# oramasearch/oramacore

Measured on NVIDIA H100. Metric: hybrid_search_qps_at_recall10_ge_0.99_1Mx768, higher is better.
Workload: dtype f32

## Files before the change

### include/oramacore_b200.h

```cpp
#ifndef ORAMACORE_B200_H
#define ORAMACORE_B200_H

#include <stddef.h>
#include <stdint.h>

#ifdef __cplusplus
extern "C" {
#endif

#define OC_OK 0
#define OC_ERR_INVALID (-1)
#define OC_ERR_CUDA (-2)
#define OC_ERR_OOM (-3)
#define OC_ERR_UNSUPPORTED (-4)
#define OC_ERR_COMM (-5)

#define OC_MAX_TOPK 1024u
#define OC_MAX_TOKENS 32u

#define OC_MODE_FULLTEXT 0
#define OC_MODE_VECTOR 1
#define OC_MODE_HYBRID 2

#define OC_DTYPE_F32 0
// ... 372 lines not shown
    float scan_ms;
    float bm25_ms;
    float fuse_ms;
    float comm_ms;
    uint32_t kernel_launches;
    uint32_t scan_launches;
    uint64_t scan_bytes;
    uint64_t bm25_postings;
    uint64_t h2d_bytes, d2h_bytes;
    uint32_t scan_tensor_core;
    uint32_t scan_unproven;
    uint32_t scan_variant;
    float scan_sweep_ms;
    float rerun_ms;
    uint32_t scan_rescored;
} oc_timing;
#define OC_SCAN_EXACT 0
#define OC_SCAN_TC_TF32 1
#define OC_SCAN_TC_BF16 4
#define OC_SCAN_TC_F16 5
int oc_last_timing(oc_ctx *ctx, oc_timing *out);
uint64_t oc_launch_count(oc_ctx *ctx);

#ifdef __cplusplus
}
#endif
#endif
```

### oramacore_b200/_lib.py

```python
from __future__ import annotations

import ctypes as C
import os
import subprocess

_HERE = os.path.dirname(os.path.abspath(__file__))
SO_PATH = os.environ.get("OC_SO_PATH") or os.path.join(_HERE, "liboramacore_b200.so")
CSRC = os.path.join(_HERE, "csrc")

OC_OK = 0
OC_MAX_TOPK = 1024
OC_COMM_ID_BYTES = 128
OC_GEO_EARTH_RADIUS_M = 6371000.0
OC_GEO_MAX_VERTICES = 2048
OC_RANGE_LO_OPEN = 1
OC_RANGE_HI_OPEN = 2
OC_FACET_UNIQUE = 1
OC_SCAN_EXACT = 0
OC_SCAN_TC_TF32 = 1
OC_SCAN_TC_BF16 = 4
OC_SCAN_TC_F16 = 5
OC_EMB_COMPACT_SHRINK = 1
OC_BATCHER_MIXED = 1
OC_WHERE_NONE, OC_WHERE_VARIANT, OC_WHERE_RANGE, OC_WHERE_GEO_RADIUS, OC_WHERE_GEO_POLYGON = 0, 1, 2, 3, 4
# ... 118 lines not shown

class ResolveQuery(C.Structure):
    _fields_ = [("exact", C.c_int), ("tolerance", C.c_int), ("field_boost", C.c_void_p), ("field_mask", C.c_void_p)]


STEM_FN = C.CFUNCTYPE(C.c_size_t, C.c_void_p, C.c_size_t, C.c_void_p, C.c_size_t, C.c_void_p)


class Timing(C.Structure):
    _fields_ = [("h2d_ms", C.c_float), ("device_ms", C.c_float), ("d2h_ms", C.c_float), ("scan_ms", C.c_float),
                ("bm25_ms", C.c_float), ("fuse_ms", C.c_float), ("comm_ms", C.c_float),
                ("kernel_launches", C.c_uint32), ("scan_launches", C.c_uint32), ("scan_bytes", C.c_uint64),
                ("bm25_postings", C.c_uint64), ("h2d_bytes", C.c_uint64), ("d2h_bytes", C.c_uint64),
                ("scan_tensor_core", C.c_uint32), ("scan_unproven", C.c_uint32),
                ("scan_variant", C.c_uint32), ("scan_sweep_ms", C.c_float), ("rerun_ms", C.c_float),
                ("scan_rescored", C.c_uint32)]

    def as_dict(self):
        return {n: getattr(self, n) for n, _ in self._fields_}


def build(force: bool = False) -> str:
    srcs = [os.path.join(CSRC, f) for f in os.listdir(CSRC) if f.endswith((".cu", ".cuh", ".h"))]
    srcs.append(os.path.join(_HERE, "..", "include", "oramacore_b200.h"))
    stale = (not os.path.exists(SO_PATH)) or any(os.path.getmtime(s) > os.path.getmtime(SO_PATH) for s in srcs)
    if force or stale:
        r = subprocess.run(["make", "-C", CSRC] + (["-B"] if force else []), capture_output=True, text=True)
        if r.returncode != 0:
            raise RuntimeError("nvcc build failed:\n" + r.stdout + r.stderr)
    return SO_PATH

# ... 160 lines not shown
```

### oramacore_b200/csrc/bm25.cuh

```cuda
#pragma once
#include "oc_common.cuh"

namespace oc {

#ifndef OC_BM25_TILE_ROWS
#define OC_BM25_TILE_ROWS 8192
#endif
constexpr uint32_t BM25_TILE = OC_BM25_TILE_ROWS;
#ifndef OC_BM25_THREADS
#define OC_BM25_THREADS 256
#endif
constexpr uint32_t BM25_THREADS = OC_BM25_THREADS;
constexpr uint32_t BM25_CHUNK = BM25_THREADS * 4;

struct PostingRaw {
    uint32_t row;
    uint16_t tf, len;
};
struct Posting {
    uint32_t row;
    float ntf;
};

struct TermDesc {
// ... 49 lines not shown
    Posting o;
    o.row = r.row;
    o.ntf = bm25_ntf(r.tf, r.len, avg, b, __fsub_rn(1.0f, b), 1.0f);
    out[i] = o;
}

__device__ __forceinline__ float bm25_sat(float S, float k, float kp1, float idf) {
    return __fdiv_rn(__fmul_rn(__fmul_rn(idf, kp1), S), __fadd_rn(k, S));
}
struct PreDesc {
    const Posting *src;
    Posting *dst;
    float *dense;
    uint32_t len;
    float weight, idf;
    uint32_t pad;
};
__device__ __forceinline__ bool f32_is_normal(float x) {
    const uint32_t e = (__float_as_uint(x) >> 23) & 0xffu;
    return e != 0u && e != 0xffu;
}

constexpr uint32_t BM25_CLASSES = 5;
struct Bm25Params {
    const TermDesc *terms;
    const TokenDesc *tokens;
    const QueryDesc *queries;
    const uint32_t *term_token;
    const uint32_t *seg;
    uint32_t n_queries, n_tiles;
    uint64_t n_rows;
// ... 12 lines not shown
    unsigned long long *tau;
    uint64_t *cand_key;
    float *cand_ft;
    uint32_t *cand_cnt;
    uint32_t *tile_count;
    float *tile_max, *tile_min;
    uint32_t tile_first;
    uint32_t *matched_bits;
    const uint32_t *perm;
    uint32_t cls_off[BM25_CLASSES];
    uint32_t cls_nq[BM25_CLASSES];
    uint32_t cls_q0[BM25_CLASSES];
    float *row_ft;
    const uint32_t *q_ok_slot;
    uint64_t ok_words;
};
__device__ __forceinline__ const uint32_t *row_ok_of(const uint32_t *bits, const uint32_t *slot, uint64_t words, uint32_t q) {
    return (bits && slot) ? bits + size_t(slot[q]) * words : bits;
}
__host__ __device__ __forceinline__ void bm25_item_decode(const Bm25Params &p, const uint32_t k, uint32_t &tile, uint32_t &q) {
    if (!p.perm) { tile = k / p.n_queries; q = k % p.n_queries; return; }
    uint32_t g = 0;
    while (g + 1 < BM25_CLASSES && k >= p.cls_off[g + 1]) g++;
    const uint32_t local = k - p.cls_off[g], nqg = p.cls_nq[g];
    tile = local / nqg;
    q = p.perm[p.cls_q0[g] + local % nqg];
}

__host__ __device__ inline size_t bm25_smem_bytes(bool multi, bool threshold, bool omc, uint32_t cap) {
    size_t b = size_t(BM25_TILE) * 4;
    if (multi || omc) b += size_t(BM25_TILE) * 4;
    if (threshold) b += size_t(BM25_TILE) * 4;
    b += size_t(BM25_TILE) / 8;
    b += size_t(cap) * 8;
    return b + 64;
}

constexpr uint32_t PRE_CHUNK = 4096;
__global__ void __launch_bounds__(256) bm25_precompute_kernel(const PreDesc *pre, const uint2 *items, float k,
                                                              const uint32_t *row_ok_bits) {
    const uint2 it = items[blockIdx.x];
    const PreDesc d = pre[it.x];
    const float kp1 = __fadd_rn(k, 1.0f);
    const uint32_t lo = it.y * PRE_CHUNK, hi = min(d.len, lo + PRE_CHUNK);
    const uint2 *src = reinterpret_cast<const uint2 *>(d.src);
    uint2 *dst = reinterpret_cast<uint2 *>(d.dst);
    for (uint32_t i = lo + threadIdx.x; i < hi; i += blockDim.x) {
        const uint2 r = __ldg(src + i);
        const float ntf = __fmul_rn(d.weight, __uint_as_float(r.y));
        float c = __int_as_float(0x7fc00000);
        if (f32_is_normal(ntf)) c = bm25_sat(ntf, k, kp1, d.idf);
        if (d.dense) {
            const bool ok = !row_ok_bits || ((row_ok_bits[r.x >> 5] >> (r.x & 31)) & 1u);
            if (ok && c == c) d.dense[r.x] = c;
        } else {
            dst[i] = make_uint2(r.x, __float_as_uint(c));
        }
    }
}

struct DfParams {
    const TermDesc *terms;
    const TokenDesc *tokens;
    uint32_t n_tokens, n_tiles;
    const uint32_t *seg;
    const uint32_t *row_ok_bits;
    unsigned int *df;
    const uint32_t *tok_ok_slot;
    uint64_t ok_words;
};
__global__ void __launch_bounds__(BM25_THREADS) bm25_df_kernel(const DfParams p) {
    __shared__ uint8_t flag[BM25_TILE];
// ... 350 lines not shown

__host__ __device__ inline size_t bm25_tile2_smem_bytes(bool threshold, bool omc, uint32_t cap) {
    size_t b = size_t(BM25_TILE) * 4;
    if (omc) b += size_t(BM25_TILE) * 4;
    if (threshold) b += size_t(BM25_TILE) * 4;
    b += size_t(BM25_TILE) / 8;
    b += size_t(cap) * 8;
    return b + 64;
}

struct ItemTok {
    const void *ptr;
    uint32_t n;
    uint32_t flags;
    float w, idf;
    uint32_t bit, pad;
};
constexpr uint32_t BM25_FLAT_TOK = 4;
__global__ void __launch_bounds__(256) bm25_flatten_kernel(const Bm25Params p, ItemTok *flat) {
    const TermDesc *terms = p.terms; const TokenDesc *tokens = p.tokens; const QueryDesc *queries = p.queries;
    const uint32_t *seg = p.seg;
    const uint32_t n_tiles = p.n_tiles, n_queries = p.n_queries;
    const uint64_t gid = uint64_t(blockIdx.x) * blockDim.x + threadIdx.x;
    const uint64_t total = uint64_t(n_tiles) * n_queries * BM25_FLAT_TOK;
    if (gid >= total) return;
    const uint32_t j = uint32_t(gid % BM25_FLAT_TOK);
    const uint64_t item = gid / BM25_FLAT_TOK;
    uint32_t tile, q;
    bm25_item_decode(p, uint32_t(item), tile, q);
    const QueryDesc qd = queries[q];
    ItemTok it{};
    if (j < qd.token_end - qd.token_begin) {
        const TokenDesc tk = tokens[qd.token_begin + j];
        it.idf = tk.idf; it.bit = tk.bit;
        if (tk.term_end > tk.term_begin) {
            const TermDesc td = terms[tk.term_begin];
            it.flags = td.flags; it.w = td.weight;
            if (td.flags & TD_DENSE) {
                it.ptr = reinterpret_cast<const float *>(td.ptr) + size_t(tile) * BM25_TILE;
                it.n = td.len ? BM25_TILE : 0;
            } else {
                const uint32_t *sg = seg + size_t(tk.term_begin) * (n_tiles + 1);
                const uint32_t lo = sg[tile], hi = sg[tile + 1];
                it.ptr = reinterpret_cast<const uint2 *>(td.ptr) + lo;
                it.n = hi - lo;
            }
        }
    }
    flat[gid] = it;
}

template <bool THRESH, bool OMC, bool ROWFT = false>
__global__ void __launch_bounds__(BM25_THREADS, 1024 / BM25_THREADS) bm25_tile2_kernel(const Bm25Params p, const ItemTok *flat, unsigned int *work_counter) {
    extern __shared__ __align__(16) uint8_t smem[];
    float *score = reinterpret_cast<float *>(smem);
// ... 331 lines not shown
    const unsigned long long key = make_key(s, row);
    if (key <= tau) return;
    const uint32_t slot = atomicAdd(s_cnt, 1u);
    if (slot < cap) tbuf[slot] = key;
}
__device__ __forceinline__ bool t3_find(const uint2 *pp, uint32_t n, uint32_t row, uint32_t *payload) {
    uint32_t lo = 0, hi = n;
    while (lo < hi) { const uint32_t m = (lo + hi) >> 1; if (__ldg(&pp[m].x) < row) lo = m + 1; else hi = m; }
    if (lo < n) { const uint2 r = __ldg(pp + lo); if (r.x == row) { *payload = r.y; return true; } }
    return false;
}
__device__ __noinline__ float t3_fold(const ItemTok *tab, const uint32_t *bm, const uint32_t j, const uint2 rec, const uint32_t l,
                                         const float k, const float kp1) {
    constexpr uint32_t W = BM25_TILE / 32;
    const uint32_t w = l >> 5, bit = 1u << (l & 31u);
    float s = 0.f;
#pragma unroll 1
    for (uint32_t i = 0; i < BM25_FLAT_TOK; i++) {
        const uint32_t ni = tab[i].n;
        if (ni == 0) continue;
        const uint32_t fi = tab[i].flags;
        float ci;
        if (fi & TD_DENSE) ci = __ldg(reinterpret_cast<const float *>(tab[i].ptr) + l);
        else {
            uint32_t pay = rec.y;
            if (i != j) {
                if (!(bm[i * W + w] & bit)) continue;
                if (!t3_find(reinterpret_cast<const uint2 *>(tab[i].ptr), ni, rec.x, &pay)) continue;
            }
            if (fi & TD_PRE) ci = __uint_as_float(pay);
            else {
                const float ntf = __fmul_rn(tab[i].w, __uint_as_float(pay));
                ci = f32_is_normal(ntf) ? bm25_sat(ntf, k, kp1, tab[i].idf) : __int_as_float(0x7fc00000);
            }
        }
        if (ci == ci) s = __fadd_rn(s, ci);
    }
    return s;
// ... 51 lines not shown
            lmax = fmaxf(lmax, m4);
            if (!pos) lmin = fminf(lmin, fminf(fminf(sv[0], sv[1]), fminf(sv[2], sv[3])));
            if (m4 >= tau_f) t3_consider4(sv[0], sv[1], sv[2], sv[3], row0 + i * 4u, tau, tau_f, s_cnt, tbuf, cap);
        }
    };
    load(ca, 0);
#pragma unroll 1
    for (uint32_t h = 0; h < NB; h += 2) {
        load(cb, h + 1);
        fold(ca, h);
        if (h + 2 < NB) load(ca, h + 2);
        fold(cb, h + 1);
    }
}

__global__ void __launch_bounds__(BM25_THREADS, 1024 / BM25_THREADS) bm25_tile3_kernel(const Bm25Params p, const ItemTok *flat, unsigned int *work_counter) {
    constexpr uint32_t W = BM25_TILE / 32;
    extern __shared__ __align__(16) uint8_t smem[];
    uint32_t *touched = reinterpret_cast<uint32_t *>(smem);
    uint32_t *bm = touched + W;
    uint64_t *tbuf = reinterpret_cast<uint64_t *>(bm + BM25_FLAT_TOK * W);
    __shared__ uint32_t s_cnt2[2], s_matched2[2];
    __shared__ unsigned int s_maxo2[2], s_mino2[2];
    __shared__ ItemTok s_tab[2][BM25_FLAT_TOK];
    __shared__ uint32_t s_item_cur, s_item_next;

    const uint32_t tid = threadIdx.x;
    const float kp1 = __fadd_rn(p.k, 1.0f);
    const uint32_t n_items = p.n_tiles * p.n_queries;
    const uint32_t *okbits = p.row_ok_bits;

    for (uint32_t i = tid; i < (BM25_FLAT_TOK + 1) * W; i += BM25_THREADS) touched[i] = 0u;
    if (tid == 0) { s_item_cur = atomicAdd(work_counter, 1u); s_item_next = atomicAdd(work_counter, 1u); }
    if (tid < 2) { s_cnt2[tid] = 0; s_matched2[tid] = 0; s_maxo2[tid] = f32_ordered(0.f); s_mino2[tid] = f32_ordered(0.f); }
    __syncthreads();
    if (s_item_cur < n_items && tid < BM25_FLAT_TOK) s_tab[0][tid] = flat[size_t(s_item_cur) * BM25_FLAT_TOK + tid];
    unsigned long long tau_next = 0ull;
    if (s_item_cur < n_items) { uint32_t t0, q0; bm25_item_decode(p, s_item_cur, t0, q0); tau_next = __ldcg(p.tau + q0); }

    for (uint32_t par = 0;; par ^= 1u) {
        __syncthreads();
        const uint32_t item = s_item_cur;
        if (item >= n_items) break;
        const uint32_t next = s_item_next;
        uint32_t next2 = 0;
        if (tid == 0) next2 = atomicAdd(work_counter, 1u);
        uint32_t tile, q;
        bm25_item_decode(p, item, tile, q);
        const uint32_t row0 = tile * BM25_TILE;
        uint32_t *s_cnt = &s_cnt2[par];
        if (tid == 0) { s_cnt2[par ^ 1u] = 0; s_matched2[par ^ 1u] = 0; s_maxo2[par ^ 1u] = f32_ordered(0.f); s_mino2[par ^ 1u] = f32_ordered(0.f); }
        ItemTok nx{};
        if (next < n_items && tid < BM25_FLAT_TOK) nx = flat[size_t(next) * BM25_FLAT_TOK + tid];
        unsigned long long tau = tau_next;
        if (next < n_items) { uint32_t tn, qn; bm25_item_decode(p, next, tn, qn); tau_next = __ldcg(p.tau + qn); }

        const ItemTok *tab = s_tab[par];
        const float4 *d0 = nullptr, *d1 = nullptr, *d2 = nullptr, *d3 = nullptr;
        uint32_t nd = 0, n_list = 0;
        bool pos = p.k >= 0.f;
#pragma unroll
        for (uint32_t j = 0; j < BM25_FLAT_TOK; j++) {
            const uint32_t n = tab[j].n;
            if (n == 0) continue;
            pos = pos && tab[j].w >= 0.f && tab[j].idf >= 0.f;
            if (tab[j].flags & TD_DENSE) {
                const float4 *dp = reinterpret_cast<const float4 *>(tab[j].ptr);
                if (nd == 0) d0 = dp; else if (nd == 1) d1 = dp; else if (nd == 2) d2 = dp; else d3 = dp;
                nd++;
            } else n_list++;
// ... 9 lines not shown
#pragma unroll 1
                for (uint32_t j = 0; j < BM25_FLAT_TOK; j++) {
                    const uint32_t n = tab[j].n;
                    if (n == 0 || (tab[j].flags & TD_DENSE)) continue;
                    const uint2 *pp = reinterpret_cast<const uint2 *>(tab[j].ptr);
                    for (uint32_t pi = tid; pi < n; pi += BM25_THREADS) {
                        const uint32_t row = __ldg(&pp[pi].x);
                        if (okbits && !((__ldg(okbits + (row >> 5)) >> (row & 31u)) & 1u)) continue;
                        const uint32_t l = row - row0, bit = 1u << (l & 31u);
                        if (nd) atomicOr(&touched[l >> 5], bit);
                        if (use_bm) atomicOr(&bm[j * W + (l >> 5)], bit);
                    }
                }
                __syncthreads();
            }
            switch (nd) {
                case 0: break;
                case 1: t3_scan<1, BM25_THREADS>(d0, d1, d2, d3, touched, any_list, pos, row0, tid, tau, tau_f, s_cnt, tbuf, p.cap, matched, lmax, lmin); break;
                case 2: t3_scan<2, BM25_THREADS>(d0, d1, d2, d3, touched, any_list, pos, row0, tid, tau, tau_f, s_cnt, tbuf, p.cap, matched, lmax, lmin); break;
                case 3: t3_scan<3, BM25_THREADS>(d0, d1, d2, d3, touched, any_list, pos, row0, tid, tau, tau_f, s_cnt, tbuf, p.cap, matched, lmax, lmin); break;
                default: t3_scan<4, BM25_THREADS>(d0, d1, d2, d3, touched, any_list, pos, row0, tid, tau, tau_f, s_cnt, tbuf, p.cap, matched, lmax, lmin); break;
            }
            if (any_list) {
#pragma unroll 1
                for (uint32_t j = 0; j < BM25_FLAT_TOK; j++) {
                    const uint32_t n = tab[j].n;
                    if (n == 0 || (tab[j].flags & TD_DENSE)) continue;
                    const uint2 *pp = reinterpret_cast<const uint2 *>(tab[j].ptr);
                    for (uint32_t pi = tid; pi < n; pi += BM25_THREADS) {
                        const uint2 rec = __ldg(pp + pi);
                        const uint32_t l = rec.x - row0, w = l >> 5, bit = 1u << (l & 31u);
// ... 45 lines not shown
            c = p.n_keep;
            if (tid == 0) atomicMax(p.tau + q, (unsigned long long)tbuf[p.n_keep - 1]);
        }
        for (uint32_t i = tid; i < c; i += BM25_THREADS) {
            const uint64_t key = tbuf[i];
            p.cand_key[slot_base * p.n_keep + i] = key;
            p.cand_ft[slot_base * p.n_keep + i] = key_score(key);
        }
        if (tid == 0) {
            p.cand_cnt[slot_base] = c;
            p.tile_count[slot_base] = s_matched2[par];
            p.tile_max[slot_base] = f32_unordered(s_maxo2[par]);
            p.tile_min[slot_base] = f32_unordered(s_mino2[par]);
        }
        if (tid < BM25_FLAT_TOK) s_tab[par ^ 1u][tid] = nx;
        if (tid == 0) { s_item_cur = next; s_item_next = next2; }
    }
}

constexpr uint32_t BW_WARPS = 6, BW_CAP = 256;
struct __align__(16) WarpScratch {
    uint32_t touched[BM25_TILE / 32];
    uint32_t bm[BM25_FLAT_TOK * (BM25_TILE / 32)];
    uint64_t tbuf[BW_CAP];
    ItemTok tab[BM25_FLAT_TOK];
    uint32_t cnt, pad[3];
};
__device__ __noinline__ unsigned long long warp_keep_top(uint64_t *buf, const uint32_t count, const uint32_t n, const uint32_t lane) {
    constexpr uint32_t PER = BW_CAP / 32;
    unsigned long long k[PER];
#pragma unroll
    for (uint32_t u = 0; u < PER; u++) k[u] = lane + 32u * u < count ? buf[lane + 32u * u] : 0ull;
    __syncwarp();
    unsigned long long mine = 0ull, last = 0ull;
    for (uint32_t r = 0; r < n; r++) {
        unsigned long long m = k[0];
#pragma unroll
        for (uint32_t u = 1; u < PER; u++) m = k[u] > m ? k[u] : m;
        for (int o = 16; o > 0; o >>= 1) {
            const unsigned long long om = __shfl_xor_sync(0xffffffffu, m, o);
            m = om > m ? om : m;
// ... 9 lines not shown
    return last;
}
__global__ void __launch_bounds__(BW_WARPS * 32, 5) bm25_warp_kernel(const Bm25Params p, const ItemTok *flat, unsigned int *work_counter) {
    constexpr uint32_t W = BM25_TILE / 32;
    extern __shared__ __align__(16) uint8_t smem[];
    const uint32_t lane = threadIdx.x & 31u;
    WarpScratch &ws = reinterpret_cast<WarpScratch *>(smem)[threadIdx.x >> 5];
    uint32_t *touched = ws.touched, *bm = ws.bm;
    const ItemTok *tab = ws.tab;
    const float kp1 = __fadd_rn(p.k, 1.0f);
    const uint32_t n_items = p.n_tiles * p.n_queries;
    const uint32_t *okbits = p.row_ok_bits;

    for (uint32_t i = lane; i < W; i += 32) touched[i] = 0u;
    for (uint32_t i = lane; i < BM25_FLAT_TOK * W; i += 32) bm[i] = 0u;
    if (lane == 0) ws.cnt = 0u;
    uint32_t item = 0, next = 0;
    if (lane == 0) { item = atomicAdd(work_counter, 1u); next = atomicAdd(work_counter, 1u); }
    item = __shfl_sync(0xffffffffu, item, 0); next = __shfl_sync(0xffffffffu, next, 0);
    ItemTok cur{};
    if (item < n_items && lane < BM25_FLAT_TOK) cur = flat[size_t(item) * BM25_FLAT_TOK + lane];
    unsigned long long tau_next = 0ull;
    if (item < n_items) { uint32_t t0, q0; bm25_item_decode(p, item, t0, q0); tau_next = __ldcg(p.tau + q0); }

    while (item < n_items) {
        uint32_t next2 = 0;
        if (lane == 0) next2 = atomicAdd(work_counter, 1u);
        uint32_t tile, q;
        bm25_item_decode(p, item, tile, q);
        const uint32_t row0 = tile * BM25_TILE;
        if (lane < BM25_FLAT_TOK) ws.tab[lane] = cur;
        ItemTok nx{};
        if (next < n_items && lane < BM25_FLAT_TOK) nx = flat[size_t(next) * BM25_FLAT_TOK + lane];
        unsigned long long tau = tau_next;
        if (next < n_items) { uint32_t tn, qn; bm25_item_decode(p, next, tn, qn); tau_next = __ldcg(p.tau + qn); }
        __syncwarp();

        const float4 *d0 = nullptr, *d1 = nullptr, *d2 = nullptr, *d3 = nullptr;
        uint32_t nd = 0, n_list = 0;
        bool pos = p.k >= 0.f;
#pragma unroll
        for (uint32_t j = 0; j < BM25_FLAT_TOK; j++) {
            const uint32_t n = tab[j].n;
            if (n == 0) continue;
            pos = pos && tab[j].w >= 0.f && tab[j].idf >= 0.f;
            if (tab[j].flags & TD_DENSE) {
                const float4 *dp = reinterpret_cast<const float4 *>(tab[j].ptr);
                if (nd == 0) d0 = dp; else if (nd == 1) d1 = dp; else if (nd == 2) d2 = dp; else d3 = dp;
                nd++;
// ... 10 lines not shown
#pragma unroll 1
                for (uint32_t j = 0; j < BM25_FLAT_TOK; j++) {
                    const uint32_t n = tab[j].n;
                    if (n == 0 || (tab[j].flags & TD_DENSE)) continue;
                    const uint2 *pp = reinterpret_cast<const uint2 *>(tab[j].ptr);
                    for (uint32_t pi = lane; pi < n; pi += 32) {
                        const uint32_t row = __ldg(&pp[pi].x);
                        if (okbits && !((__ldg(okbits + (row >> 5)) >> (row & 31u)) & 1u)) continue;
                        const uint32_t l = row - row0, bit = 1u << (l & 31u);
                        if (nd) atomicOr(&touched[l >> 5], bit);
                        if (use_bm) atomicOr(&bm[j * W + (l >> 5)], bit);
                    }
                }
                __syncwarp();
            }
            switch (nd) {
                case 0: break;
                case 1: t3_scan<1, 32>(d0, d1, d2, d3, touched, any_list, pos, row0, lane, tau, tau_f, &ws.cnt, ws.tbuf, BW_CAP, matched, lmax, lmin); break;
                case 2: t3_scan<2, 32>(d0, d1, d2, d3, touched, any_list, pos, row0, lane, tau, tau_f, &ws.cnt, ws.tbuf, BW_CAP, matched, lmax, lmin); break;
                case 3: t3_scan<3, 32>(d0, d1, d2, d3, touched, any_list, pos, row0, lane, tau, tau_f, &ws.cnt, ws.tbuf, BW_CAP, matched, lmax, lmin); break;
                default: t3_scan<4, 32>(d0, d1, d2, d3, touched, any_list, pos, row0, lane, tau, tau_f, &ws.cnt, ws.tbuf, BW_CAP, matched, lmax, lmin); break;
            }
            if (any_list) {
#pragma unroll 1
                for (uint32_t j = 0; j < BM25_FLAT_TOK; j++) {
                    const uint32_t n = tab[j].n;
                    if (n == 0 || (tab[j].flags & TD_DENSE)) continue;
                    const uint2 *pp = reinterpret_cast<const uint2 *>(tab[j].ptr);
                    for (uint32_t pi = lane; pi < n; pi += 32) {
                        const uint2 rec = __ldg(pp + pi);
                        const uint32_t l = rec.x - row0, w = l >> 5, bit = 1u << (l & 31u);
// ... 47 lines not shown
            p.tile_count[slot_base] = matched;
            p.tile_max[slot_base] = lmax;
            p.tile_min[slot_base] = lmin;
            ws.cnt = 0u;
        }
        if (lane < BM25_FLAT_TOK && nx.n) {
            const char *pf = reinterpret_cast<const char *>(nx.ptr);
            const uint32_t bytes = (nx.flags & TD_DENSE) ? 1024u : min(nx.n * 8u, 1024u);
            for (uint32_t o = 0; o < bytes; o += 128u) asm volatile("prefetch.global.L1 [%0];" ::"l"(pf + o));
        }
        cur = nx;
        item = next;
        next = __shfl_sync(0xffffffffu, next2, 0);
        __syncwarp();
    }
}

struct PointParams {
    const TermDesc *terms; const TokenDesc *tokens; const QueryDesc *queries;
    uint32_t n_queries, v_stride;
    const uint32_t *v_row;
    const uint32_t *row_ok_bits;
    float k;
    int threshold;
    float *v_ft; uint8_t *v_present;
    const uint32_t *q_ok_slot;
    uint64_t ok_words;
};
__device__ __forceinline__ bool posting_find(const TermDesc &td, uint32_t row, uint32_t *payload) {
    const uint2 *pp = reinterpret_cast<const uint2 *>(td.ptr);
// ... 134 lines not shown
```

### oramacore_b200/csrc/capi.cu

```cuda
#include <cuda_runtime.h>

#include <cub/device/device_radix_sort.cuh>
#include <cub/device/device_scan.cuh>

#include <algorithm>
#include <atomic>
#include <chrono>
#include <cmath>
#include <cstdarg>
#include <cstdio>
#include <cstring>
#include <limits>
#include <map>
#include <memory>
#include <mutex>
#include <utility>
#include <string>
#include <unordered_map>
#include <unordered_set>
#include <vector>

#include "bm25.cuh"
#include "comm.h"
#include "dense_cache.h"
// ... 2494 lines not shown
    Slot<FacetSliceDev> s_fslices;
    Slot<TermDesc> s_terms;
    Slot<TokenDesc> s_tokens;
    Slot<QueryDesc> s_queries;
    Slot<PreDesc> s_pre;
    Slot<SortEntry> s_sent;
    Slot<SortQuery> s_sq;
    Slot<uint8_t> s_salt;
    Bm25Params bp{};
    FuseParams fp{};
    size_t fuse_smem = 0;
    const uint32_t *row_ok = nullptr;
    float *min_hint_dev = nullptr;
    unsigned int *tile_counter = nullptr;
    bool did_comm = false;
    size_t o_sc = 0, o_n = 0, o_cnt = 0, o_min = 0, o_gflag = 0, out_bytes = 0, o_resc = 0;
    uint8_t *dout = nullptr;
    uint64_t *d_doc = nullptr;
    float *d_score = nullptr;
    uint32_t *d_n = nullptr;
};

static int upload(const Packer &pk, HostBuf &hb, DevBuf &db, cudaStream_t st) {
    OCTRY(hb.ensure(pk.total + 256));
    OCTRY(db.ensure(pk.total + 256));
    pk.fill(hb.p);
    size_t run0 = 0;
    for (size_t i = 0; i <= pk.segs.size(); i++) {
        const bool brk = i == pk.segs.size() || pk.segs[i].direct;
        if (brk) {
            const size_t end = i == pk.segs.size() ? pk.total : pk.segs[i].off;
// ... 324 lines not shown
        size_t slot = (h ^ (h >> 29)) & (cap_t - 1);
        while (tab_v[slot] != 0xffffffffu && !(tab_k[slot].a == key.a && tab_k[slot].b == key.b)) slot = (slot + 1) & (cap_t - 1);
        if (tab_v[slot] == 0xffffffffu) {
            tab_k[slot] = key; tab_v[slot] = (uint32_t)uniq.size();
            uniq.push_back({e, 0, key}); distinct += terms[e].len;
        }
        uniq[tab_v[slot]].uses++;
        e_to_u[e] = tab_v[slot];
        walked += terms[e].len;
    }
    const char *share_env = getenv("OC_BM25_SHARE");
    const bool share_off = share_env && !strcmp(share_env, "off"), share_force = share_env && !strcmp(share_env, "force");
    const char *dense_env = getenv("OC_BM25_DENSE");
    const char *t2_env = getenv("OC_BM25_TILE2");
    const bool dense_on = !k.any_multi && !(dense_env && dense_env[0] == '0') && !share_off && !(t2_env && t2_env[0] == '0');
    const uint64_t rows_pad = uint64_t(k.n_tiles) * BM25_TILE;
    const uint64_t dense_min = std::max<uint64_t>(512, k.S->n_rows / 16);
    std::vector<uint8_t> u_dense(uniq.size(), 0);
    uint64_t n_dense = 0;
    if (dense_on)
        for (size_t u = 0; u < uniq.size(); u++)
            if (terms[uniq[u].first_e].len >= dense_min && (n_dense + 1) * rows_pad * 4 <= (size_t(8) << 30)) { u_dense[u] = 1; n_dense++; }
    uint64_t walked_l = 0, distinct_l = 0;
    for (size_t e = 0; e < terms.size(); e++)
        if (e_to_u[e] != 0xffffffffu && !u_dense[e_to_u[e]]) walked_l += terms[e].len;
    for (size_t u = 0; u < uniq.size(); u++) if (!u_dense[u]) distinct_l += terms[uniq[u].first_e].len;
    const bool lists = distinct_l && !share_off && (share_force || (walked_l >= 2 * distinct_l && walked_l >= (64u << 20))) &&
                       distinct_l * 8 <= (size_t(6) << 30);
    if (!lists && !n_dense) return OC_OK;
    std::vector<float *> u_arr(uniq.size(), nullptr);
    std::vector<uint8_t> u_kept(uniq.size(), 0);
    if (n_dense) {
        std::vector<DenseKey> keys;
        std::vector<uint32_t> key_u;
        uint32_t kb, bb;
        memcpy(&kb, &k.p->bm25_k, 4); memcpy(&bb, &k.p->bm25_b, 4);
        for (size_t u = 0; u < uniq.size(); u++)
            if (u_dense[u]) {
                keys.push_back(DenseKey{k.S->ident, uniq[u].key.a, uint32_t(uniq[u].key.b >> 32), uint32_t(uniq[u].key.b), kb, bb});
                key_u.push_back((uint32_t)u);
            }
        std::vector<float *> arr;
        std::vector<uint8_t> build;
        dense_cache_bind(k, keys, rows_pad * 4, arr, build);
        for (size_t i = 0; i < keys.size(); i++) { u_arr[key_u[i]] = arr[i]; u_kept[key_u[i]] = arr[i] && !build[i]; }
    }
    uint64_t n_buf = 0;
    for (size_t u = 0; u < uniq.size(); u++) n_buf += u_dense[u] && !u_arr[u];
    if (lists) OCTRY(c->pre_post.ensure(distinct_l * 8 + 64));
    if (n_buf) OCTRY(c->dense_buf.ensure(n_buf * rows_pad * 4));
    k.dense_bytes = n_buf * rows_pad * 4;
    uint64_t off = 0, doff = 0;
    std::vector<uint64_t> u_off(uniq.size());
    std::vector<uint8_t> u_used(uniq.size(), 0);
    for (size_t u = 0; u < uniq.size(); u++) {
        if (!u_dense[u] && !lists) continue;
        u_used[u] = 1;
        if (u_dense[u] && !u_arr[u]) { u_arr[u] = c->dense_buf.as<float>() + doff; doff += rows_pad; }
        if (u_kept[u]) continue;
        const TermDesc &td = terms[uniq[u].first_e];
        PreDesc pd{};
        pd.src = td.ptr; pd.len = td.len; pd.weight = td.weight;
        pd.idf = tokens[k.term_token[uniq[u].first_e]].idf;
        if (u_dense[u]) pd.dense = u_arr[u];
        else { u_off[u] = off; pd.dst = c->pre_post.as<Posting>() + off; off += td.len; }
        const uint32_t pi = (uint32_t)k.pre_descs.size();
        k.pre_descs.push_back(pd);
        for (uint32_t ch = 0; ch * PRE_CHUNK < td.len; ch++) k.pre_items.push_back(make_uint2(pi, ch));
    }
    for (size_t e = 0; e < terms.size(); e++) {
        const uint32_t u = e_to_u[e];
        if (u == 0xffffffffu || !u_used[u]) continue;
        if (u_dense[u]) { terms[e].ptr = reinterpret_cast<const Posting *>(u_arr[u]); terms[e].flags |= TD_DENSE; }
        else { terms[e].ptr = c->pre_post.as<Posting>() + u_off[u]; terms[e].flags |= TD_PRE; }
    }
    return OC_OK;
}

static void bm25_item_order(SearchCall &k) {
// ... 245 lines not shown
    if (k.pin_items) {
        pj->d_doc = s_pdoc.at(din);
        pj->d_pos = s_ppos.at(din);
        pj->d_cnt = s_pcnt.at(din);
    }
    const uint32_t n_keep = k.n_keep;
    k.cap = n_keep <= 32 ? std::max<uint32_t>(n_keep + BM25_CHUNK, BM25_SPARSE_MAX)
                         : next_pow2(std::max<uint32_t>(n_keep + BM25_CHUNK, BM25_SPARSE_MAX));
    k.o_sc = size_t(B) * k.limit * 8;
    k.o_n = k.o_sc + size_t(B) * k.limit * 4;
    k.o_cnt = (k.o_n + size_t(B) * 4 + 7) & ~size_t(7);
    k.o_min = k.o_cnt + size_t(B) * 8;
    k.o_gflag = k.o_min + size_t(B) * 4;
    k.out_bytes = k.o_gflag + ((size_t(B) + 3) & ~size_t(3));
    k.o_resc = k.out_bytes + ((size_t(B) + 3) & ~size_t(3));
    OCTRY(c->out_blob.ensure(k.out_bytes));
    OCTRY(c->h_out.ensure(k.o_resc + size_t(B) * 4));
    k.dout = c->out_blob.as<uint8_t>();
    k.d_doc = c->out_blob.as<uint64_t>();
    k.d_score = reinterpret_cast<float *>(k.dout + k.o_sc);
    k.d_n = reinterpret_cast<uint32_t *>(k.dout + k.o_n);
    return OC_OK;
}

static int bm25_stage(SearchCall &k) {
    oc_ctx *c = k.c; const oc_search_params *p = k.p;
    const uint32_t B = k.B, n_tiles = k.n_tiles, n_keep = k.n_keep; const StrSnap *S = k.S;
    const DevBuf &din = c->in_blob; cudaStream_t ps = k.side ? c->side : c->stream;
    CU(cudaEventRecord(c->ev[EV_BM0], ps));
    const uint64_t ok_words = uint64_t(n_tiles) * (BM25_TILE / 32);
    if (k.per_q) {
        OCTRY(c->row_ok.ensure(std::max<uint64_t>(ok_words, 1) * k.qfj.slots.size() * 4));
// ... 77 lines not shown
    bp.row_ok_bits = k.row_ok;
    if (k.per_q) { bp.q_ok_slot = k.qfj.d_q_slot_ft; bp.ok_words = ok_words; }
    bp.omc_row = p->omc ? k.omc_row_dev : k.s_omcr.at(din);
    bp.omc_mult = p->omc ? k.omc_row_mult_dev : k.s_omcrm.at(din);
    bp.n_omc = k.n_omc_rows;
    bp.v_row = nullptr;
    bp.v_stride = k.vlimit;
    bp.v_ft = nullptr; bp.v_present = nullptr;
    bp.min_hint = k.min_hint_dev;
    bp.n_keep = n_keep; bp.cap = k.cap;
    bp.tau = c->tau.as<unsigned long long>();
    bp.cand_key = c->cand_key.as<uint64_t>(); bp.cand_ft = c->cand_ft.as<float>();
    bp.cand_cnt = c->cand_cnt.as<uint32_t>(); bp.tile_count = c->tile_cnt.as<uint32_t>();
    bp.tile_max = c->tile_max.as<float>(); bp.tile_min = c->tile_min.as<float>();
    bp.tile_first = 0;
    if (!k.q_perm.empty()) {
        bp.perm = k.s_perm.at(din);
        uint32_t off = 0, q0 = 0;
        for (uint32_t g = 0; g < BM25_CLASSES; g++) {
            bp.cls_off[g] = off; bp.cls_nq[g] = k.cls_nq[g]; bp.cls_q0[g] = q0;
            off += k.cls_nq[g] * n_tiles; q0 += k.cls_nq[g];
        }
    }
    const SearchReq &r = k.r;
    if (r.fj || r.gj || r.sj) {
        OCTRY(c->mbits.ensure(size_t(B) * std::max<uint32_t>(n_tiles, 1) * (BM25_TILE / 32) * 4));
        bp.matched_bits = c->mbits.as<uint32_t>();
    }
    if (r.gj && n_tiles) {
        OCTRY(c->row_ft.ensure(size_t(B) * n_tiles * BM25_TILE * 4));
// ... 212 lines not shown
    CU(cudaEventRecord(c->ev[EV_FUSE0], c->stream));
    OCTRY(fuse_or_merge(k));
    CU(cudaEventRecord(c->ev[EV_FUSE1], c->stream));
    return OC_OK;
}

static int rerun_checks(SearchCall &k) {
    oc_ctx *c = k.c; const oc_search_params *p = k.p;
    const uint32_t B = k.B; uint8_t *h = c->h_out.as<uint8_t>();
    CU(cudaEventRecord(c->ev[EV_DEV], c->stream));
    CU(cudaMemcpyAsync(h, k.dout, k.out_bytes, cudaMemcpyDeviceToHost, c->stream));
    if (c->gemm_pending) {
        CU(cudaMemcpyAsync(h + k.out_bytes, c->g_flag.p, k.Bv, cudaMemcpyDeviceToHost, c->stream));
        CU(cudaMemcpyAsync(h + k.o_resc, c->g_resc.p, size_t(k.Bv) * 4, cudaMemcpyDeviceToHost, c->stream));
    }
    CU(cudaEventRecord(c->ev[EV_D2H], c->stream));
    CU(cudaStreamSynchronize(c->stream));
    {
        bool rerun = false;
        if (k.did_comm && k.has_v) for (uint32_t q = 0; q < B; q++) rerun = rerun || h[k.o_gflag + q] != 0;
        uint32_t redone = 0;
        if (c->gemm_pending || rerun) CU(cudaEventRecord(c->ev[EV_RR0], c->stream));
        if (c->gemm_pending) {
            const uint32_t Bv = k.Bv;
            uint64_t resc = 0;
            for (uint32_t q = 0; q < Bv; q++) resc += reinterpret_cast<const uint32_t *>(h + k.o_resc)[q];
            c->timing.scan_rescored = (uint32_t)(resc / Bv);
            OCTRY(fix_unproven(c, k.emb, h + k.out_bytes, Bv, k.vlimit, p->similarity, &redone));
        }
        if (redone || rerun) {
            c->gemm_pending = false;
            OCTRY(device_tail(k));
// ... 2172 lines not shown
```

Before: 159,500.

## Skip dense BM25 tile scans using per-tile score upper bounds and hit bitmaps

While building the dense BM25 term arrays, the precompute kernel now also records a nonzero bitmap and a per-tile maximum contribution. In the tile kernels, when the sum of dense bounds for a tile is below the query's current threshold tau, the full dense score scan is replaced by a popcount over the bitmaps to keep the match count. This avoids reading and scoring dense float arrays for tiles that cannot enter the top-k. The cost is extra atomics and memory during precompute, plus a stats readback. The tau handling also moves into shared memory.

```diff
diff --git a/include/oramacore_b200.h b/include/oramacore_b200.h
--- a/include/oramacore_b200.h
+++ b/include/oramacore_b200.h
@@ -410,6 +410,8 @@
     float scan_sweep_ms;
     float rerun_ms;
     uint32_t scan_rescored;
+    uint32_t bm25_dense_items;
+    uint32_t bm25_dense_skipped;
 } oc_timing;
 #define OC_SCAN_EXACT 0
 #define OC_SCAN_TC_TF32 1
diff --git a/oramacore_b200/_lib.py b/oramacore_b200/_lib.py
--- a/oramacore_b200/_lib.py
+++ b/oramacore_b200/_lib.py
@@ -156,7 +156,7 @@
                 ("bm25_postings", C.c_uint64), ("h2d_bytes", C.c_uint64), ("d2h_bytes", C.c_uint64),
                 ("scan_tensor_core", C.c_uint32), ("scan_unproven", C.c_uint32),
                 ("scan_variant", C.c_uint32), ("scan_sweep_ms", C.c_float), ("rerun_ms", C.c_float),
-                ("scan_rescored", C.c_uint32)]
+                ("scan_rescored", C.c_uint32), ("bm25_dense_items", C.c_uint32), ("bm25_dense_skipped", C.c_uint32)]
 
     def as_dict(self):
         return {n: getattr(self, n) for n, _ in self._fields_}
diff --git a/oramacore_b200/csrc/bm25.cuh b/oramacore_b200/csrc/bm25.cuh
--- a/oramacore_b200/csrc/bm25.cuh
+++ b/oramacore_b200/csrc/bm25.cuh
@@ -87,7 +87,7 @@
     float *dense;
     uint32_t len;
     float weight, idf;
-    uint32_t pad;
+    uint32_t n_tiles;
 };
 __device__ __forceinline__ bool f32_is_normal(float x) {
     const uint32_t e = (__float_as_uint(x) >> 23) & 0xffu;
@@ -130,6 +130,7 @@
     float *row_ft;
     const uint32_t *q_ok_slot;
     uint64_t ok_words;
+    uint32_t *dense_stat;
 };
 __device__ __forceinline__ const uint32_t *row_ok_of(const uint32_t *bits, const uint32_t *slot, uint64_t words, uint32_t q) {
     return (bits && slot) ? bits + size_t(slot[q]) * words : bits;
@@ -152,6 +153,16 @@
     return b + 64;
 }
 
+__host__ __device__ inline uint64_t bm25_dense_bytes(uint32_t n_tiles) {
+    const uint64_t rows_pad = uint64_t(n_tiles) * BM25_TILE;
+    return rows_pad * 4 + rows_pad / 8 + ((uint64_t(n_tiles) * 4 + 255) & ~uint64_t(255));
+}
+__host__ __device__ __forceinline__ const uint32_t *bm25_dense_bits(const float *arr, uint32_t n_tiles) {
+    return reinterpret_cast<const uint32_t *>(arr + size_t(n_tiles) * BM25_TILE);
+}
+__host__ __device__ __forceinline__ const float *bm25_dense_bound(const float *arr, uint32_t n_tiles) {
+    return reinterpret_cast<const float *>(bm25_dense_bits(arr, n_tiles) + size_t(n_tiles) * (BM25_TILE / 32));
+}
 constexpr uint32_t PRE_CHUNK = 4096;
 __global__ void __launch_bounds__(256) bm25_precompute_kernel(const PreDesc *pre, const uint2 *items, float k,
                                                               const uint32_t *row_ok_bits) {
@@ -160,18 +171,40 @@
     const float kp1 = __fadd_rn(k, 1.0f);
     const uint32_t lo = it.y * PRE_CHUNK, hi = min(d.len, lo + PRE_CHUNK);
     const uint2 *src = reinterpret_cast<const uint2 *>(d.src);
-    uint2 *dst = reinterpret_cast<uint2 *>(d.dst);
-    for (uint32_t i = lo + threadIdx.x; i < hi; i += blockDim.x) {
-        const uint2 r = __ldg(src + i);
-        const float ntf = __fmul_rn(d.weight, __uint_as_float(r.y));
-        float c = __int_as_float(0x7fc00000);
-        if (f32_is_normal(ntf)) c = bm25_sat(ntf, k, kp1, d.idf);
-        if (d.dense) {
+    if (!d.dense) {
+        uint2 *dst = reinterpret_cast<uint2 *>(d.dst);
+        for (uint32_t i = lo + threadIdx.x; i < hi; i += blockDim.x) {
+            const uint2 r = __ldg(src + i);
+            const float ntf = __fmul_rn(d.weight, __uint_as_float(r.y));
+            float c = __int_as_float(0x7fc00000);
+            if (f32_is_normal(ntf)) c = bm25_sat(ntf, k, kp1, d.idf);
+            dst[i] = make_uint2(r.x, __float_as_uint(c));
+        }
+        return;
+    }
+    uint32_t *bits = const_cast<uint32_t *>(bm25_dense_bits(d.dense, d.n_tiles));
+    unsigned int *bound = reinterpret_cast<unsigned int *>(const_cast<float *>(bm25_dense_bound(d.dense, d.n_tiles)));
+    const uint32_t lane = threadIdx.x & 31u;
+    for (uint32_t i0 = lo + (threadIdx.x - lane); i0 < hi; i0 += blockDim.x) {
+        const uint32_t i = i0 + lane;
+        uint32_t row = 0, v = 0;
+        if (i < hi) {
+            const uint2 r = __ldg(src + i);
+            const float ntf = __fmul_rn(d.weight, __uint_as_float(r.y));
+            float c = __int_as_float(0x7fc00000);
+            if (f32_is_normal(ntf)) c = bm25_sat(ntf, k, kp1, d.idf);
             const bool ok = !row_ok_bits || ((row_ok_bits[r.x >> 5] >> (r.x & 31)) & 1u);
-            if (ok && c == c) d.dense[r.x] = c;
-        } else {
-            dst[i] = make_uint2(r.x, __float_as_uint(c));
-        }
+            row = r.x;
+            if (ok && c == c) {
+                d.dense[row] = c;
+                if (c != 0.f) atomicOr(bits + (row >> 5), 1u << (row & 31u));
+                if (c > 0.f) v = __float_as_uint(c);
+            }
+        }
+        const uint32_t tile = row / BM25_TILE;
+        const uint32_t grp = __match_any_sync(0xffffffffu, tile);
+        const uint32_t m = __reduce_max_sync(grp, v);
+        if (m && lane == uint32_t(__ffs(grp) - 1)) atomicMax(bound + tile, m);
     }
 }
 
@@ -552,7 +585,8 @@
     uint32_t n;
     uint32_t flags;
     float w, idf;
-    uint32_t bit, pad;
+    uint32_t bit;
+    uint32_t bound;
 };
 constexpr uint32_t BM25_FLAT_TOK = 4;
 __global__ void __launch_bounds__(256) bm25_flatten_kernel(const Bm25Params p, ItemTok *flat) {
@@ -577,6 +611,7 @@
             if (td.flags & TD_DENSE) {
                 it.ptr = reinterpret_cast<const float *>(td.ptr) + size_t(tile) * BM25_TILE;
                 it.n = td.len ? BM25_TILE : 0;
+                if (td.len) it.bound = __float_as_uint(bm25_dense_bound(reinterpret_cast<const float *>(td.ptr), n_tiles)[tile]);
             } else {
                 const uint32_t *sg = seg + size_t(tk.term_begin) * (n_tiles + 1);
                 const uint32_t lo = sg[tile], hi = sg[tile + 1];
@@ -938,6 +973,11 @@
                                          const float k, const float kp1) {
     constexpr uint32_t W = BM25_TILE / 32;
     const uint32_t w = l >> 5, bit = 1u << (l & 31u);
+    static_assert(BM25_FLAT_TOK == 4, "t3_fold holds one dense contribution per flat token");
+    auto dense_at = [&](const uint32_t i) {
+        return (tab[i].n && (tab[i].flags & TD_DENSE)) ? __ldg(reinterpret_cast<const float *>(tab[i].ptr) + l) : 0.f;
+    };
+    const float cd0 = dense_at(0), cd1 = dense_at(1), cd2 = dense_at(2), cd3 = dense_at(3);
     float s = 0.f;
 #pragma unroll 1
     for (uint32_t i = 0; i < BM25_FLAT_TOK; i++) {
@@ -945,7 +985,7 @@
         if (ni == 0) continue;
         const uint32_t fi = tab[i].flags;
         float ci;
-        if (fi & TD_DENSE) ci = __ldg(reinterpret_cast<const float *>(tab[i].ptr) + l);
+        if (fi & TD_DENSE) ci = i == 0 ? cd0 : i == 1 ? cd1 : i == 2 ? cd2 : cd3;
         else {
             uint32_t pay = rec.y;
             if (i != j) {
@@ -1027,6 +1067,35 @@
     }
 }
 
+__device__ __forceinline__ float t3_dense_ub(const ItemTok *tab) {
+    float ub = 0.f;
+#pragma unroll
+    for (uint32_t j = 0; j < BM25_FLAT_TOK; j++)
+        if (tab[j].n && (tab[j].flags & TD_DENSE)) ub = __fadd_rn(ub, __uint_as_float(tab[j].bound));
+    return ub;
+}
+template <uint32_t STRIDE>
+__device__ __noinline__ uint32_t t3_count(const ItemTok *tab, const uint32_t *touched, const bool any_list, const uint32_t n_tiles,
+                                          const uint32_t tile, const uint32_t tid) {
+    constexpr uint32_t W = BM25_TILE / 32;
+    const uint32_t *bp[BM25_FLAT_TOK];
+#pragma unroll
+    for (uint32_t j = 0; j < BM25_FLAT_TOK; j++)
+        bp[j] = (tab[j].n && (tab[j].flags & TD_DENSE))
+                    ? bm25_dense_bits(reinterpret_cast<const float *>(tab[j].ptr) - size_t(tile) * BM25_TILE, n_tiles) + size_t(tile) * W
+                    : nullptr;
+    uint32_t m = 0;
+#pragma unroll 2
+    for (uint32_t w = tid; w < W; w += STRIDE) {
+        uint32_t u = 0;
+#pragma unroll
+        for (uint32_t j = 0; j < BM25_FLAT_TOK; j++) if (bp[j]) u |= __ldg(bp[j] + w);
+        if (any_list) u &= ~touched[w];
+        m += __popc(u);
+    }
+    return m;
+}
+
 __global__ void __launch_bounds__(BM25_THREADS, 1024 / BM25_THREADS) bm25_tile3_kernel(const Bm25Params p, const ItemTok *flat, unsigned int *work_counter) {
     constexpr uint32_t W = BM25_TILE / 32;
     extern __shared__ __align__(16) uint8_t smem[];
@@ -1037,6 +1106,8 @@
     __shared__ unsigned int s_maxo2[2], s_mino2[2];
     __shared__ ItemTok s_tab[2][BM25_FLAT_TOK];
     __shared__ uint32_t s_item_cur, s_item_next;
+    __shared__ uint32_t s_dense[2];
+    __shared__ unsigned long long s_tau2[2];
 
     const uint32_t tid = threadIdx.x;
     const float kp1 = __fadd_rn(p.k, 1.0f);
@@ -1044,12 +1115,15 @@
     const uint32_t *okbits = p.row_ok_bits;
 
     for (uint32_t i = tid; i < (BM25_FLAT_TOK + 1) * W; i += BM25_THREADS) touched[i] = 0u;
-    if (tid == 0) { s_item_cur = atomicAdd(work_counter, 1u); s_item_next = atomicAdd(work_counter, 1u); }
+    if (tid == 0) { s_item_cur = atomicAdd(work_counter, 1u); s_item_next = atomicAdd(work_counter, 1u); s_dense[0] = s_dense[1] = 0u; }
     if (tid < 2) { s_cnt2[tid] = 0; s_matched2[tid] = 0; s_maxo2[tid] = f32_ordered(0.f); s_mino2[tid] = f32_ordered(0.f); }
     __syncthreads();
     if (s_item_cur < n_items && tid < BM25_FLAT_TOK) s_tab[0][tid] = flat[size_t(s_item_cur) * BM25_FLAT_TOK + tid];
     unsigned long long tau_next = 0ull;
-    if (s_item_cur < n_items) { uint32_t t0, q0; bm25_item_decode(p, s_item_cur, t0, q0); tau_next = __ldcg(p.tau + q0); }
+    if (tid == 0) {
+        s_tau2[0] = 0ull;
+        if (s_item_cur < n_items) { uint32_t t0, q0; bm25_item_decode(p, s_item_cur, t0, q0); s_tau2[0] = __ldcg(p.tau + q0); }
+    }
 
     for (uint32_t par = 0;; par ^= 1u) {
         __syncthreads();
@@ -1065,8 +1139,8 @@
         if (tid == 0) { s_cnt2[par ^ 1u] = 0; s_matched2[par ^ 1u] = 0; s_maxo2[par ^ 1u] = f32_ordered(0.f); s_mino2[par ^ 1u] = f32_ordered(0.f); }
         ItemTok nx{};
         if (next < n_items && tid < BM25_FLAT_TOK) nx = flat[size_t(next) * BM25_FLAT_TOK + tid];
-        unsigned long long tau = tau_next;
-        if (next < n_items) { uint32_t tn, qn; bm25_item_decode(p, next, tn, qn); tau_next = __ldcg(p.tau + qn); }
+        unsigned long long tau = s_tau2[par];
+        if (tid == 0 && next < n_items) { uint32_t tn, qn; bm25_item_decode(p, next, tn, qn); tau_next = __ldcg(p.tau + qn); }
 
         const ItemTok *tab = s_tab[par];
         const float4 *d0 = nullptr, *d1 = nullptr, *d2 = nullptr, *d3 = nullptr;
@@ -1106,7 +1180,10 @@
                 }
                 __syncthreads();
             }
-            switch (nd) {
+            const bool skip = nd && pos && t3_dense_ub(tab) < tau_f;
+            if (nd && tid == 0) { s_dense[0]++; s_dense[1] += skip; }
+            if (skip) matched += t3_count<BM25_THREADS>(tab, touched, any_list, p.n_tiles, tile, tid);
+            else switch (nd) {
                 case 0: break;
                 case 1: t3_scan<1, BM25_THREADS>(d0, d1, d2, d3, touched, any_list, pos, row0, tid, tau, tau_f, s_cnt, tbuf, p.cap, matched, lmax, lmin); break;
                 case 2: t3_scan<2, BM25_THREADS>(d0, d1, d2, d3, touched, any_list, pos, row0, tid, tau, tau_f, s_cnt, tbuf, p.cap, matched, lmax, lmin); break;
@@ -1182,8 +1259,9 @@
             p.tile_min[slot_base] = f32_unordered(s_mino2[par]);
         }
         if (tid < BM25_FLAT_TOK) s_tab[par ^ 1u][tid] = nx;
-        if (tid == 0) { s_item_cur = next; s_item_next = next2; }
-    }
+        if (tid == 0) { s_item_cur = next; s_item_next = next2; s_tau2[par ^ 1u] = tau_next; }
+    }
+    if (tid == 0 && p.dense_stat && s_dense[0]) { atomicAdd(p.dense_stat, s_dense[0]); atomicAdd(p.dense_stat + 1, s_dense[1]); }
 }
 
 constexpr uint32_t BW_WARPS = 6, BW_CAP = 256;
@@ -1192,7 +1270,7 @@
     uint32_t bm[BM25_FLAT_TOK * (BM25_TILE / 32)];
     uint64_t tbuf[BW_CAP];
     ItemTok tab[BM25_FLAT_TOK];
-    uint32_t cnt, pad[3];
+    uint32_t cnt, dense_items, dense_skipped, pad;
 };
 __device__ __noinline__ unsigned long long warp_keep_top(uint64_t *buf, const uint32_t count, const uint32_t n, const uint32_t lane) {
     constexpr uint32_t PER = BW_CAP / 32;
@@ -1232,7 +1310,7 @@
 
     for (uint32_t i = lane; i < W; i += 32) touched[i] = 0u;
     for (uint32_t i = lane; i < BM25_FLAT_TOK * W; i += 32) bm[i] = 0u;
-    if (lane == 0) ws.cnt = 0u;
+    if (lane == 0) { ws.cnt = 0u; ws.dense_items = 0u; ws.dense_skipped = 0u; }
     uint32_t item = 0, next = 0;
     if (lane == 0) { item = atomicAdd(work_counter, 1u); next = atomicAdd(work_counter, 1u); }
     item = __shfl_sync(0xffffffffu, item, 0); next = __shfl_sync(0xffffffffu, next, 0);
@@ -1250,7 +1328,7 @@
         if (lane < BM25_FLAT_TOK) ws.tab[lane] = cur;
         ItemTok nx{};
         if (next < n_items && lane < BM25_FLAT_TOK) nx = flat[size_t(next) * BM25_FLAT_TOK + lane];
-        unsigned long long tau = tau_next;
+        unsigned long long tau = __shfl_sync(0xffffffffu, tau_next, 0);
         if (next < n_items) { uint32_t tn, qn; bm25_item_decode(p, next, tn, qn); tau_next = __ldcg(p.tau + qn); }
         __syncwarp();
 
@@ -1291,7 +1369,10 @@
                 }
                 __syncwarp();
             }
-            switch (nd) {
+            const bool skip = nd && pos && t3_dense_ub(tab) < tau_f;
+            if (nd && lane == 0) { ws.dense_items++; ws.dense_skipped += skip; }
+            if (skip) matched += t3_count<32>(tab, touched, any_list, p.n_tiles, tile, lane);
+            else switch (nd) {
                 case 0: break;
                 case 1: t3_scan<1, 32>(d0, d1, d2, d3, touched, any_list, pos, row0, lane, tau, tau_f, &ws.cnt, ws.tbuf, BW_CAP, matched, lmax, lmin); break;
                 case 2: t3_scan<2, 32>(d0, d1, d2, d3, touched, any_list, pos, row0, lane, tau, tau_f, &ws.cnt, ws.tbuf, BW_CAP, matched, lmax, lmin); break;
@@ -1369,6 +1450,7 @@
         next = __shfl_sync(0xffffffffu, next2, 0);
         __syncwarp();
     }
+    if (lane == 0 && p.dense_stat && ws.dense_items) { atomicAdd(p.dense_stat, ws.dense_items); atomicAdd(p.dense_stat + 1, ws.dense_skipped); }
 }
 
 struct PointParams {
diff --git a/oramacore_b200/csrc/capi.cu b/oramacore_b200/csrc/capi.cu
--- a/oramacore_b200/csrc/capi.cu
+++ b/oramacore_b200/csrc/capi.cu
@@ -2532,7 +2532,7 @@
     float *min_hint_dev = nullptr;
     unsigned int *tile_counter = nullptr;
     bool did_comm = false;
-    size_t o_sc = 0, o_n = 0, o_cnt = 0, o_min = 0, o_gflag = 0, out_bytes = 0, o_resc = 0;
+    size_t o_sc = 0, o_n = 0, o_cnt = 0, o_min = 0, o_gflag = 0, out_bytes = 0, o_resc = 0, o_dstat = 0;
     uint8_t *dout = nullptr;
     uint64_t *d_doc = nullptr;
     float *d_score = nullptr;
@@ -2887,13 +2887,13 @@
     const char *dense_env = getenv("OC_BM25_DENSE");
     const char *t2_env = getenv("OC_BM25_TILE2");
     const bool dense_on = !k.any_multi && !(dense_env && dense_env[0] == '0') && !share_off && !(t2_env && t2_env[0] == '0');
-    const uint64_t rows_pad = uint64_t(k.n_tiles) * BM25_TILE;
+    const uint64_t dbytes = bm25_dense_bytes(k.n_tiles);
     const uint64_t dense_min = std::max<uint64_t>(512, k.S->n_rows / 16);
     std::vector<uint8_t> u_dense(uniq.size(), 0);
     uint64_t n_dense = 0;
     if (dense_on)
         for (size_t u = 0; u < uniq.size(); u++)
-            if (terms[uniq[u].first_e].len >= dense_min && (n_dense + 1) * rows_pad * 4 <= (size_t(8) << 30)) { u_dense[u] = 1; n_dense++; }
+            if (terms[uniq[u].first_e].len >= dense_min && (n_dense + 1) * dbytes <= (size_t(8) << 30)) { u_dense[u] = 1; n_dense++; }
     uint64_t walked_l = 0, distinct_l = 0;
     for (size_t e = 0; e < terms.size(); e++)
         if (e_to_u[e] != 0xffffffffu && !u_dense[e_to_u[e]]) walked_l += terms[e].len;
@@ -2915,27 +2915,27 @@
             }
         std::vector<float *> arr;
         std::vector<uint8_t> build;
-        dense_cache_bind(k, keys, rows_pad * 4, arr, build);
+        dense_cache_bind(k, keys, dbytes, arr, build);
         for (size_t i = 0; i < keys.size(); i++) { u_arr[key_u[i]] = arr[i]; u_kept[key_u[i]] = arr[i] && !build[i]; }
     }
     uint64_t n_buf = 0;
     for (size_t u = 0; u < uniq.size(); u++) n_buf += u_dense[u] && !u_arr[u];
     if (lists) OCTRY(c->pre_post.ensure(distinct_l * 8 + 64));
-    if (n_buf) OCTRY(c->dense_buf.ensure(n_buf * rows_pad * 4));
-    k.dense_bytes = n_buf * rows_pad * 4;
+    if (n_buf) OCTRY(c->dense_buf.ensure(n_buf * dbytes));
+    k.dense_bytes = n_buf * dbytes;
     uint64_t off = 0, doff = 0;
     std::vector<uint64_t> u_off(uniq.size());
     std::vector<uint8_t> u_used(uniq.size(), 0);
     for (size_t u = 0; u < uniq.size(); u++) {
         if (!u_dense[u] && !lists) continue;
         u_used[u] = 1;
-        if (u_dense[u] && !u_arr[u]) { u_arr[u] = c->dense_buf.as<float>() + doff; doff += rows_pad; }
+        if (u_dense[u] && !u_arr[u]) { u_arr[u] = c->dense_buf.as<float>() + doff; doff += dbytes / 4; }
         if (u_kept[u]) continue;
         const TermDesc &td = terms[uniq[u].first_e];
         PreDesc pd{};
         pd.src = td.ptr; pd.len = td.len; pd.weight = td.weight;
         pd.idf = tokens[k.term_token[uniq[u].first_e]].idf;
-        if (u_dense[u]) pd.dense = u_arr[u];
+        if (u_dense[u]) { pd.dense = u_arr[u]; pd.n_tiles = k.n_tiles; }
         else { u_off[u] = off; pd.dst = c->pre_post.as<Posting>() + off; off += td.len; }
         const uint32_t pi = (uint32_t)k.pre_descs.size();
         k.pre_descs.push_back(pd);
@@ -3211,8 +3211,9 @@
     k.o_gflag = k.o_min + size_t(B) * 4;
     k.out_bytes = k.o_gflag + ((size_t(B) + 3) & ~size_t(3));
     k.o_resc = k.out_bytes + ((size_t(B) + 3) & ~size_t(3));
+    k.o_dstat = k.o_resc + size_t(B) * 4;
     OCTRY(c->out_blob.ensure(k.out_bytes));
-    OCTRY(c->h_out.ensure(k.o_resc + size_t(B) * 4));
+    OCTRY(c->h_out.ensure(k.o_dstat + 8));
     k.dout = c->out_blob.as<uint8_t>();
     k.d_doc = c->out_blob.as<uint64_t>();
     k.d_score = reinterpret_cast<float *>(k.dout + k.o_sc);
@@ -3320,6 +3321,7 @@
     bp.cand_cnt = c->cand_cnt.as<uint32_t>(); bp.tile_count = c->tile_cnt.as<uint32_t>();
     bp.tile_max = c->tile_max.as<float>(); bp.tile_min = c->tile_min.as<float>();
     bp.tile_first = 0;
+    bp.dense_stat = k.tile_counter + 2;
     if (!k.q_perm.empty()) {
         bp.perm = k.s_perm.at(din);
         uint32_t off = 0, q0 = 0;
@@ -3562,8 +3564,12 @@
         CU(cudaMemcpyAsync(h + k.out_bytes, c->g_flag.p, k.Bv, cudaMemcpyDeviceToHost, c->stream));
         CU(cudaMemcpyAsync(h + k.o_resc, c->g_resc.p, size_t(k.Bv) * 4, cudaMemcpyDeviceToHost, c->stream));
     }
+    const bool dstat = k.has_ft && k.n_tiles;
+    if (dstat) CU(cudaMemcpyAsync(h + k.o_dstat, k.tile_counter + 2, 8, cudaMemcpyDeviceToHost, c->stream));
     CU(cudaEventRecord(c->ev[EV_D2H], c->stream));
     CU(cudaStreamSynchronize(c->stream));
+    c->timing.bm25_dense_items = dstat ? reinterpret_cast<const uint32_t *>(h + k.o_dstat)[0] : 0u;
+    c->timing.bm25_dense_skipped = dstat ? reinterpret_cast<const uint32_t *>(h + k.o_dstat)[1] : 0u;
     {
         bool rerun = false;
         if (k.did_comm && k.has_v) for (uint32_t q = 0; q < B; q++) rerun = rerun || h[k.o_gflag + q] != 0;
```

After: 176,000, median of 6. +10.4%, better.
